# b1xian/arm-neon-opencv

Hardware: AMD Instinct MI355X
Metric: Mpixels/sec per op (resize/warp/normalize) at 1080p; achieved HBM GB/s vs peak (higher is better)
Workload: dtype u8; 1 GPU; resize_normalize INTER_LINEAR 1920x1080x3 u8 NHWC -> 640x360x3 fp32 (reference arithmetic) + per-channel normalize; global_batch=256, batch_per_gpu=256, parallelism=dp1, frame=1920x1080x3, output=640x360x3 fp32, graph=False

## Files before the change

### arm-neon-opencv_amd/csrc/vacv_abi.cpp

```cpp
#pragma clang fp contract(off)

#include <hip/hip_runtime.h>

#include <algorithm>
#include <cfloat>
#include <cmath>
#include <cstdint>
#include <cstdlib>
#include <cstring>
#include <map>
#include <set>
#include <mutex>
#include <tuple>
#include <utility>

#include "vacv_internal.hpp"
#include "vacv_semantics.hpp"

namespace vacv {
namespace {

int esize_of(int dtype) {
    switch (dtype) {
        case VACV_FP32: return 4;
        case VACV_FP16: return 2;
        case VACV_INT8: return 1;
        case VACV_FP64: return 8;
        default: return 0;
    }
}

struct Img {
    unsigned char* data;
    int n, w, h, c, dtype, layout, es;
    int64_t row, plane, batch;
};

int load(const vacv_image* d, Img& m) {
    if (!d || !d->data) return VACV_ERR_INVALID_ARG;
    if (d->n < 1 || d->w < 1 || d->h < 1 || d->c < 1) return VACV_ERR_INVALID_ARG;
    m.es = esize_of(d->dtype);
    if (!m.es) return VACV_ERR_UNSUPPORTED;
    if (d->layout != VACV_NHWC && d->layout != VACV_NCHW) return VACV_ERR_UNSUPPORTED;
    m.data = static_cast<unsigned char*>(d->data);
    m.n = d->n; m.w = d->w; m.h = d->h; m.c = d->c;
    m.dtype = d->dtype; m.layout = d->layout;
    const int64_t min_row = (int64_t)m.w * (m.layout == VACV_NHWC ? m.c : 1) * m.es;
    m.row = d->row_pitch ? d->row_pitch : min_row;
    if (m.row < min_row) return VACV_ERR_INVALID_ARG;
    if (m.layout == VACV_NCHW) {
        const int64_t min_plane = m.row * (m.h - 1) + min_row;
        m.plane = d->plane_pitch ? d->plane_pitch : m.row * m.h;
        if (m.plane < min_plane) return VACV_ERR_INVALID_ARG;
        const int64_t min_batch = m.plane * (m.c - 1) + min_plane;
        m.batch = d->batch_pitch ? d->batch_pitch : m.plane * m.c;
        if (m.n > 1 && m.batch < min_batch) return VACV_ERR_INVALID_ARG;
    } else {
        m.plane = 0;
        const int64_t min_batch = m.row * (m.h - 1) + min_row;
        m.batch = d->batch_pitch ? d->batch_pitch : m.row * m.h;
        if (m.n > 1 && m.batch < min_batch) return VACV_ERR_INVALID_ARG;
    }
    return VACV_OK;
}

int load2(const vacv_image* src_d, const vacv_image* dst_d, Img& src, Img& dst) {
    const int st = load(src_d, src);
    return st ? st : load(dst_d, dst);
}

bool dense(const Img& m) {
    const int64_t row = (int64_t)m.w * (m.layout == VACV_NHWC ? m.c : 1) * m.es;
    if (m.row != row) return false;
    if (m.layout == VACV_NCHW && m.plane != row * m.h) return false;
    const int64_t img = row * m.h * (m.layout == VACV_NCHW ? m.c : 1);
    return m.n == 1 || m.batch == img;
}

PlaneGeom geom(const Img& m) {
    PlaneGeom g;
    g.base = m.data;
    g.img_pitch = m.batch;
    g.row_pitch = m.row;
    g.w = m.w;
    g.h = m.h;
    g.esize = m.es;
    if (m.layout == VACV_NHWC) {
        g.planes = 1;
        g.cc = m.c;
        g.plane_pitch = 0;
    } else {
        g.planes = m.c;
        g.cc = 1;
        g.plane_pitch = m.plane;
    }
    g.plane_bytes = m.row * (m.h - 1) + (int64_t)m.w * g.cc * m.es;
    return g;
}

int hip_status(hipError_t e) { return e == hipSuccess ? VACV_OK : VACV_ERR_HIP; }

bool same_shape(const Img& a, const Img& b) {
    return a.n == b.n && a.w == b.w && a.h == b.h && a.c == b.c && a.layout == b.layout;
}

struct Workspace {
    void* buf = nullptr;
    size_t cap = 0;
};
std::mutex g_ws_mu;
std::map<std::tuple<int, void*, int>, Workspace> g_ws;

int workspace(hipStream_t s, size_t bytes, void** out, int slot = 0, bool zero_new = false) {
    int dev = 0;
    if (hipGetDevice(&dev) != hipSuccess) return VACV_ERR_HIP;
    std::lock_guard<std::mutex> lk(g_ws_mu);
    Workspace& w = g_ws[std::make_tuple(dev, (void*)s, slot)];
    if (w.cap < bytes) {
        if (w.buf) {
            if (hipStreamSynchronize(s) != hipSuccess) return VACV_ERR_HIP;
            (void)hipFree(w.buf);
            w.buf = nullptr;
            w.cap = 0;
        }
        size_t cap = std::max<size_t>(bytes, 1 << 20);
        if (hipMalloc(&w.buf, cap) != hipSuccess) return VACV_ERR_NO_MEMORY;
        w.cap = cap;
        if (zero_new && hipMemsetAsync(w.buf, 0, cap, s) != hipSuccess) return VACV_ERR_HIP;
    }
    *out = w.buf;
    return VACV_OK;
}

size_t align_up(size_t v, size_t a) { return (v + a - 1) / a * a; }

int channel_sums_into(const Img& m, double* sums, int per_image, double* partials, int blocks, hipStream_t s) {
    SumsLaunch L{};
    L.src = geom(m);
    L.n = m.n;
    L.c = m.c;
    L.src_u8 = m.dtype == VACV_INT8;
    L.blocks_per_image = blocks;
    L.partials = partials;
    L.sums = sums;
    L.per_image = per_image;
    L.scalar_only = 0;
    for (int i = 0; i < m.n && !L.scalar_only; ++i)
        for (int p = 0; p < L.src.planes; ++p) {
            uintptr_t a = reinterpret_cast<uintptr_t>(m.data + (int64_t)i * m.batch + (int64_t)p * L.src.plane_pitch);
            if (a & 15) { L.scalar_only = 1; break; }
        }
    return hip_status(launch_channel_sums(L, s));
}

int sums_blocks(const Img& m) {
    const int64_t elems = (int64_t)m.w * m.h * (m.layout == VACV_NHWC ? m.c : 1);
    const int64_t planes = (int64_t)m.n * (m.layout == VACV_NHWC ? 1 : m.c);
    int64_t b = std::max<int64_t>(1, 2048 / std::max<int64_t>(planes, 1));
    b = std::min<int64_t>(b, std::max<int64_t>(1, elems / 4096));
    return (int)std::min<int64_t>(b, 1024);
}

int per_image_stats(const Img& m, hipStream_t s, float** mean, float** stdv) {
    if (m.layout == VACV_NHWC && m.c > 4) return VACV_ERR_UNSUPPORTED;
    if (!dense(m)) return VACV_ERR_UNSUPPORTED;
    const int blocks = sums_blocks(m);
    const int planes = m.layout == VACV_NHWC ? 1 : m.c;
    const int cc = m.layout == VACV_NHWC ? m.c : 1;
    const size_t part_b = align_up((size_t)m.n * planes * blocks * 2 * cc * sizeof(double), 256);
    const size_t sums_b = align_up((size_t)m.n * m.c * 2 * sizeof(double), 256);
    const size_t stat_b = align_up((size_t)m.n * m.c * sizeof(float), 256);
    void* ws = nullptr;
    int st = workspace(s, part_b + sums_b + 2 * stat_b, &ws);
    if (st) return st;
    char* p = static_cast<char*>(ws);
    double* partials = reinterpret_cast<double*>(p);
    double* sums = reinterpret_cast<double*>(p + part_b);
    *mean = reinterpret_cast<float*>(p + part_b + sums_b);
    *stdv = reinterpret_cast<float*>(p + part_b + sums_b + stat_b);
    st = channel_sums_into(m, sums, 1, partials, blocks, s);
    if (st) return st;
    return hip_status(launch_stats(sums, m.n, m.c, (double)m.w * m.h, *mean, *stdv, s));
}

int norm_spec(const Img& shape, const float* mean, const float* stdv, NormSpec& ns) {
    std::memset(&ns, 0, sizeof(ns));
    ns.c_total = shape.c;
    if (!mean && !stdv) return VACV_OK;
    if (!mean || !stdv) return VACV_ERR_INVALID_ARG;
    if (shape.c > kMaxC) return VACV_ERR_UNSUPPORTED;
    ns.mode = 1;
    ns.mul_ok = 0;
    ns.f32_ok = 0;
    for (int k = 0; k < shape.c; ++k) {
        ns.mean[k] = mean[k];
        ns.stdv[k] = stdv[k];
        ns.inv[k] = 1.0 / ((double)stdv[k] + 1e-6);
        ns.inv_hi[k] = (float)ns.inv[k];
        ns.inv_lo[k] = (float)(ns.inv[k] - (double)ns.inv_hi[k]);
        bool ok = true, ok32 = true;
        for (int v = 0; v < 256; ++v) {
            const float d = (float)v - mean[k];
            const float want = normalize_value((float)v, mean[k], stdv[k]);
            ok = ok && (float)((double)d * ns.inv[k]) == want;
            const float lo = d * ns.inv_lo[k];
            const float got = std::fma(d, ns.inv_hi[k], lo);
            ok32 = ok32 && std::memcmp(&got, &want, sizeof(float)) == 0;
        }
        if (ok) ns.mul_ok |= 1u << k;
        if (ok32) ns.f32_ok |= 1u << k;
    }
    return VACV_OK;
}

int normalize_with(const Img& src, const Img& dst, const NormSpec& ns, hipStream_t s) {
    NormLaunch L{};
    L.src = geom(src);
    L.dst = geom(dst);
    L.n = src.n;
    L.src_u8 = src.dtype == VACV_INT8;
    L.norm = ns;
    return hip_status(launch_normalize(L, s));
}

struct FusedSums {
    double* partials;
    double* sums;
    int per_image;
    float* mean;
    float* stddev;
    int groups;
    bool used;
    int64_t* acc;
};

int resolve_out(const Img& src, const Img& dst, int out_kind, int& out) {
    out = (src.dtype == VACV_FP32 && out_kind == kOutF32) ? kOutSame : out_kind;
    const int want = out == kOutSame ? src.dtype : VACV_FP32;
    return dst.dtype == want ? VACV_OK : VACV_ERR_INVALID_ARG;
}

int resize_impl(const vacv_image* src_d, const vacv_image* dst_d, int interpolation, int mode, int out_kind,
                const NormSpec* ns, hipStream_t s, double fx = 0.0, double fy = 0.0, FusedSums* fs = nullptr) {
    Img src, dst;
    int st = load2(src_d, dst_d, src, dst);
    if (st) return st;
    if (src.n != dst.n || src.c != dst.c || src.layout != dst.layout) return VACV_ERR_INVALID_ARG;
    if (src.layout == VACV_NHWC && src.c > 4) return VACV_ERR_UNSUPPORTED;
    if (mode < VACV_LINEAR_REFERENCE || mode > VACV_LINEAR_OPENCV) return VACV_ERR_INVALID_ARG;

    ResizeLaunch L{};
    L.src = geom(src);
    L.dst = geom(dst);
    if (L.src.plane_bytes > kMaxPlaneBytes || L.dst.plane_bytes > kMaxPlaneBytes) return VACV_ERR_UNSUPPORTED;
    L.n = src.n;
    L.mode = mode;
    L.out = out_kind;
    if (ns) L.norm = *ns;
    if (interpolation == VACV_INTER_LINEAR) {
        if (src.w < 2 || src.h < 2) return VACV_ERR_INVALID_ARG;
        if (src.dtype == VACV_INT8) {
            L.kind = kLinearFixed;
            const int want = out_kind == kOutSame ? VACV_INT8 : VACV_FP32;
            if (dst.dtype != want) return VACV_ERR_INVALID_ARG;
        } else if (src.dtype == VACV_FP32) {
            L.kind = kLinearFloat;
            if (dst.dtype != VACV_FP32) return VACV_ERR_INVALID_ARG;
            if (out_kind == kOutF32) L.out = kOutSame;
        } else {
            return VACV_ERR_UNSUPPORTED;
        }
    } else if (interpolation == VACV_INTER_CUBIC) {
        if (src.w < 4 || src.h < 4) return VACV_ERR_INVALID_ARG;
        if (src.dtype != VACV_INT8 && src.dtype != VACV_FP32) return VACV_ERR_UNSUPPORTED;
        if (dst.dtype != VACV_FP32) return VACV_ERR_UNSUPPORTED;
        L.kind = kCubic;
        if (L.out == kOutSame && src.dtype == VACV_INT8) L.out = kOutF32;
        if (L.out == kOutF32 && src.dtype == VACV_FP32) L.out = kOutSame;
    } else if (interpolation == VACV_INTER_NEAREST) {
        if (src.dtype != VACV_INT8 && src.dtype != VACV_FP32) return VACV_ERR_UNSUPPORTED;
        if ((st = resolve_out(src, dst, out_kind, L.out))) return st;
        L.scale_xd = 1. / (fx > 0 ? fx : (double)dst.w / src.w);
        L.scale_yd = 1. / (fy > 0 ? fy : (double)dst.h / src.h);
        return hip_status(launch_resize_nearest(L, s));
    } else if (interpolation == VACV_INTER_AREA) {
        if (src.dtype != VACV_INT8 && src.dtype != VACV_FP32) return VACV_ERR_UNSUPPORTED;
        if ((st = resolve_out(src, dst, out_kind, L.out))) return st;
        const double ifx = fx > 0 ? fx : (double)dst.w / src.w, ify = fy > 0 ? fy : (double)dst.h / src.h;
        const double sx = 1. / ifx, sy = 1. / ify;
        const double ix = std::nearbyint(sx), iy = std::nearbyint(sy);
        if (sx >= 1 && sy >= 1 && std::fabs(sx - ix) < DBL_EPSILON && std::fabs(sy - iy) < DBL_EPSILON) {
            L.area_x = (int)ix;
            L.area_y = (int)iy;
            if ((int64_t)dst.w * L.area_x != src.w || (int64_t)dst.h * L.area_y != src.h) return VACV_ERR_UNSUPPORTED;
            L.area_scale = 1.f / (float)(L.area_x * L.area_y);
            L.area_half_up = src.dtype == VACV_INT8 && L.area_x == 2 && L.area_y == 2 &&
                             (L.src.cc == 1 || L.src.cc == 3 || L.src.cc == 4);
            return hip_status(launch_resize_area(L, s));
        }
        return launch_resize_area_general(L, ifx, ify, s);
    } else if (interpolation == VACV_INTER_LANCZOS4) {
        if (src.dtype != VACV_INT8 && src.dtype != VACV_FP32) return VACV_ERR_UNSUPPORTED;
        if ((st = resolve_out(src, dst, out_kind, L.out))) return st;
        const double ifx = fx > 0 ? fx : (double)dst.w / src.w, ify = fy > 0 ? fy : (double)dst.h / src.h;
        return launch_resize_lanczos(L, ifx, ify, s);
    } else {
        return VACV_ERR_UNSUPPORTED;
    }
    L.scale_xf = (float)src.w / (float)dst.w;
    L.scale_yf = (float)src.h / (float)dst.h;
    L.scale_xd = (double)src.w / (double)dst.w;
    L.scale_yd = (double)src.h / (double)dst.h;
    const int direct = tune_or(VACV_TUNE_RESIZE_DIRECT, 1);
    if (L.kind == kLinearFixed && L.src.cc <= 4 && dst.w < (1 << 23) && dst.h < (1 << 23) &&
        (direct == 2 || ((direct == 1 || direct == 3) && resize_one_tap_rows(L))))
        return hip_status(launch_resize_direct(L, s));
    if (L.kind == kLinearFixed && tune_or(VACV_TUNE_RESIZE_STRIP, 1) >= 1 && resize_strip_applies(L))
        return hip_status(launch_resize_strip(L, s));
    if (cubic_direct_applies(L)) {
        if (fs && L.out == kOutF32 && fs->partials && L.src.planes == 1) {
            L.sum_partials = fs->partials;
            L.sum_out = fs->sums;
            L.sum_per_image = fs->per_image;
            L.sum_mean = fs->mean;
            L.sum_std = fs->stddev;
            L.sum_acc = fs->acc;
            fs->groups = cubic_direct_groups(L);
            fs->used = true;
        }
        return hip_status(launch_cubic_direct(L, s));
    }
    L.interleave = tune(VACV_TUNE_RESIZE_INTERLEAVE) != 0;
    if ((st = plan_resize(L, s))) return st;
    return hip_status(launch_resize(L, s));
}

int copy_rows(const Img& src, const Img& dst, int64_t src_off, int rows_h, int64_t row_bytes, hipStream_t s) {
    CopyLaunch L{};
    L.src = geom(src);
    L.dst = geom(dst);
    L.src.base += src_off;
    L.src.h = rows_h;
    L.n = src.n;
    L.row_bytes = row_bytes;
    return hip_status(launch_row_copy(L, s));
}

int clone_rows(const Img& src, const Img& dst, hipStream_t s) {
    const int cc = src.layout == VACV_NHWC ? src.c : 1;
    return copy_rows(src, dst, 0, src.h, (int64_t)src.w * cc * src.es, s);
}

int dtype_convert(const Img& src, const Img& dst, hipStream_t s) {
    if (!dense(src) || !dense(dst)) return VACV_ERR_UNSUPPORTED;
    DtypeLaunch L{};
    L.src = src.data;
    L.dst = dst.data;
    L.count = (int64_t)src.n * src.w * src.h * src.c;
    L.to_f32 = src.dtype == VACV_INT8;
    return hip_status(launch_dtype(L, s));
}

int border_values(const Img& src, const double* bv, float out[4]) {
    for (int k = 0; k < 4; ++k) {
        const double v = bv ? bv[k] : 0.0;
        if (src.dtype == VACV_INT8) {
            double r = std::nearbyint(v);
            out[k] = (float)std::min(255.0, std::max(0.0, r));
        } else {
            out[k] = (float)v;
        }
    }
    return VACV_OK;
}

int warp_impl(const vacv_image* src_d, const vacv_image* dst_d, const float m[6], int flags, int border_mode,
              const double bv[4], int out_kind, const NormSpec* ns, hipStream_t s) {
    Img src, dst;
    int st = load2(src_d, dst_d, src, dst);
    if (st) return st;
    if (!m) return VACV_ERR_INVALID_ARG;
    if (src.n != dst.n || src.c != dst.c || src.layout != dst.layout) return VACV_ERR_INVALID_ARG;
    if (src.dtype != VACV_INT8 && src.dtype != VACV_FP32) return VACV_ERR_UNSUPPORTED;
    const int interp = flags & 7;
    const bool inverse_map = (flags & VACV_WARP_INVERSE_MAP) != 0;
    if (flags & ~(7 | VACV_WARP_INVERSE_MAP)) return VACV_ERR_UNSUPPORTED;
    if (interp != VACV_INTER_LINEAR && interp != VACV_INTER_NEAREST) return VACV_ERR_UNSUPPORTED;
    if (border_mode < VACV_BORDER_CONSTANT || border_mode > VACV_BORDER_TRANSPARENT) return VACV_ERR_UNSUPPORTED;
    if (src.layout == VACV_NHWC && src.c > 4) return VACV_ERR_UNSUPPORTED;
    if (interp == VACV_INTER_LINEAR && (src.w < 2 || src.h < 2)) return VACV_ERR_INVALID_ARG;
    WarpLaunch L{};
    L.src = geom(src);
    L.dst = geom(dst);
    L.n = src.n;
    if ((st = resolve_out(src, dst, out_kind, L.out))) return st;
    if (inverse_map) std::memcpy(L.inv, m, sizeof(L.inv));
    else vacv_invert_affine(m, L.inv);
    border_values(src, bv, L.border);
    L.border_mode = border_mode;
    if (border_mode == VACV_BORDER_TRANSPARENT && dst.data == src.data) return VACV_ERR_INVALID_ARG;
    if (ns) L.norm = *ns;
    if (interp == VACV_INTER_NEAREST) {
        double* M = L.invd;
        for (int i = 0; i < 6; ++i) M[i] = (double)m[i];
        if (!inverse_map) {
            double D = M[0] * M[4] - M[1] * M[3];
            D = D != 0 ? 1. / D : 0;
            const double A11 = M[4] * D, A22 = M[0] * D;
            M[0] = A11;
            M[1] *= -D;
            M[3] *= -D;
            M[4] = A22;
            const double b1 = -M[0] * M[2] - M[1] * M[5];
            const double b2 = -M[3] * M[2] - M[4] * M[5];
            M[2] = b1;
            M[5] = b2;
        }
        return hip_status(launch_warp_nearest(L, s));
    }
    return hip_status(launch_warp(L, s));
}

int warp_rois_impl(const vacv_image* src_d, const vacv_image* dst_d, const float* m, const int32_t* src_index,
                   int flags, int border_mode, const double bv[4], const NormSpec* ns, hipStream_t s) {
    Img src, dst;
    int st = load2(src_d, dst_d, src, dst);
    if (st) return st;
    if (!m) return VACV_ERR_INVALID_ARG;
    if (src.c != dst.c) return VACV_ERR_INVALID_ARG;
    if (!src_index && src.n != 1 && src.n != dst.n) return VACV_ERR_INVALID_ARG;
    if (src.dtype != VACV_INT8 && src.dtype != VACV_FP32) return VACV_ERR_UNSUPPORTED;
    if (src.layout != VACV_NHWC) return VACV_ERR_UNSUPPORTED;
    if (flags & ~(7 | VACV_WARP_INVERSE_MAP)) return VACV_ERR_UNSUPPORTED;
    if ((flags & 7) != VACV_INTER_LINEAR) return VACV_ERR_UNSUPPORTED;
    if (border_mode < VACV_BORDER_CONSTANT || border_mode >= VACV_BORDER_TRANSPARENT) return VACV_ERR_UNSUPPORTED;
    if (src.c > 4) return VACV_ERR_UNSUPPORTED;
    if (src.w < 2 || src.h < 2) return VACV_ERR_INVALID_ARG;
    if (dst.dtype != (ns ? VACV_FP32 : src.dtype)) return VACV_ERR_INVALID_ARG;
    if (!ns && dst.layout != VACV_NHWC) return VACV_ERR_INVALID_ARG;
    const bool planar = dst.layout == VACV_NCHW && dst.c > 1;
    if (planar && dst.c != 3) return VACV_ERR_UNSUPPORTED;
    WarpRoisLaunch L{};
    L.src = geom(src);
    if (L.src.plane_bytes > kMaxPlaneBytes) return VACV_ERR_UNSUPPORTED;
    L.dst = geom(dst);
    L.n_src = src.n;
    L.n_roi = dst.n;
    L.m = m;
    L.src_index = src_index;
    L.inverse_map = (flags & VACV_WARP_INVERSE_MAP) != 0;
    border_values(src, bv, L.border);
    L.border_mode = border_mode;
    L.out = ns ? kOutNorm : kOutSame;
    L.planar = planar;
    if (ns) L.norm = *ns;
    return hip_status(launch_warp_rois(L, s));
}

int color_code(int code, int& v_first, int& rgb) {
    switch (code) {
        case VACV_COLOR_YUV2BGR_NV21: v_first = 1; rgb = 0; return VACV_OK;
        case VACV_COLOR_YUV2RGB_NV21: v_first = 1; rgb = 1; return VACV_OK;
        case VACV_COLOR_YUV2BGR_NV12: v_first = 0; rgb = 0; return VACV_OK;
        case VACV_COLOR_YUV2RGB_NV12: v_first = 0; rgb = 1; return VACV_OK;
        default: return VACV_ERR_UNSUPPORTED;
    }
}

int color_impl(const vacv_image* src_d, const vacv_image* dst_d, int code, int out_kind, const NormSpec* ns,
               hipStream_t s) {
    Img src, dst;
    int st = load2(src_d, dst_d, src, dst);
    if (st) return st;
    int v_first, rgb;
    if ((st = color_code(code, v_first, rgb))) return st;
    if (src.dtype != VACV_INT8 || src.c != 1) return VACV_ERR_INVALID_ARG;
    const int h = src.h / 3 * 2;
    if (src.w % 2 || h % 2 || h < 2 || src.h != h / 2 * 3) return VACV_ERR_INVALID_ARG;
    if (dst.w != src.w || dst.h != h || dst.c != 3 || dst.layout != VACV_NHWC || dst.n != src.n)
        return VACV_ERR_INVALID_ARG;
    const int want = out_kind == kOutSame ? VACV_INT8 : VACV_FP32;
    if (dst.dtype != want) return VACV_ERR_INVALID_ARG;
    ColorLaunch L{};
    L.src = src.data;
    L.src_img = src.batch;
    L.src_row = src.row;
    L.dst = dst.data;
    L.dst_img = dst.batch;
    L.dst_row = dst.row;
    L.n = src.n;
    L.w = src.w;
    L.h = h;
    L.v_first = v_first;
    L.rgb = rgb;
    L.out = out_kind;
    if (ns) L.norm = *ns;
    return hip_status(launch_color(L, s));
}

int color_cv_impl(const vacv_image* src_d, const vacv_image* dst_d, int code, hipStream_t s) {
    Img src, dst;
    int st = load2(src_d, dst_d, src, dst);
    if (st) return st;
    if (src.layout != VACV_NHWC || dst.layout != VACV_NHWC || src.c != 1 || dst.n != src.n) return VACV_ERR_INVALID_ARG;
    CvColorLaunch L{};
    L.src = src.data;
    L.src_img = src.batch;
    L.src_row = src.row;
    L.dst = dst.data;
    L.dst_img = dst.batch;
    L.dst_row = dst.row;
    L.n = src.n;
    L.w = src.w;
    if (code == VACV_COLOR_GRAY2BGR) {
        if (src.dtype != VACV_INT8 && src.dtype != VACV_FP32) return VACV_ERR_UNSUPPORTED;
        if (dst.dtype != src.dtype || dst.w != src.w || dst.h != src.h || dst.c != 3) return VACV_ERR_INVALID_ARG;
        if (src.es == 4 && ((src.row | dst.row | src.batch | dst.batch) % 4 ||
                            reinterpret_cast<uintptr_t>(src.data) % 4 || reinterpret_cast<uintptr_t>(dst.data) % 4))
            return VACV_ERR_INVALID_ARG;
        L.gray = 1;
        L.h = src.h;
        L.dcn = 3;
        L.esize = src.es;
        return hip_status(launch_color_cv(L, s));
    }
    if (src.dtype != VACV_INT8 || dst.dtype != VACV_INT8) return VACV_ERR_INVALID_ARG;
    const int h = src.h / 3 * 2;
    if (src.w % 2 || h % 2 || h < 2 || src.h != h / 2 * 3) return VACV_ERR_INVALID_ARG;
    L.h = h;
    switch (code) {
        case VACV_COLOR_YUV2RGBA_NV12: L.layout = 0; L.dcn = 4; L.bidx = 2; break;
        case VACV_COLOR_YUV2BGRA_NV12: L.layout = 0; L.dcn = 4; L.bidx = 0; break;
        case VACV_COLOR_YUV2RGBA_NV21: L.layout = 1; L.dcn = 4; L.bidx = 2; break;
        case VACV_COLOR_YUV2BGRA_NV21: L.layout = 1; L.dcn = 4; L.bidx = 0; break;
        default: L.layout = 2; L.dcn = 3; L.bidx = 0; break;
    }
    if (L.layout == 2 && src.row != src.w) return VACV_ERR_INVALID_ARG;
    if (dst.w != src.w || dst.h != h || dst.c != L.dcn) return VACV_ERR_INVALID_ARG;
    const int al = L.dcn == 4 ? 8 : 2;
    L.aligned = !((dst.row | dst.batch) % al) && !(reinterpret_cast<uintptr_t>(dst.data) % al);
    return hip_status(launch_color_cv(L, s));
}

int yuv_resize_impl(const vacv_image* src_d, const vacv_image* dst_d, int code, int interpolation, int mode,
                    int out_kind, const NormSpec* ns, hipStream_t s) {
    Img src, dst;
    int st = load2(src_d, dst_d, src, dst);
    if (st) return st;
    int v_first, rgb;
    if ((st = color_code(code, v_first, rgb))) return st;
    if (interpolation != VACV_INTER_LINEAR) return VACV_ERR_UNSUPPORTED;
    if (mode < VACV_LINEAR_REFERENCE || mode > VACV_LINEAR_OPENCV) return VACV_ERR_INVALID_ARG;
    if (src.dtype != VACV_INT8 || src.c != 1 || src.layout != VACV_NHWC) return VACV_ERR_INVALID_ARG;
    const int h = src.h / 3 * 2;
    if (src.w % 2 || h % 2 || h < 2 || src.w < 4 || src.h != h / 2 * 3) return VACV_ERR_INVALID_ARG;
    if (dst.c != 3 || dst.n != src.n) return VACV_ERR_INVALID_ARG;
    const int want = out_kind == kOutSame ? VACV_INT8 : VACV_FP32;
    if (dst.dtype != want) return VACV_ERR_INVALID_ARG;
    const int64_t src_bytes = src.row * (src.h - 1) + src.w;
    const int64_t P = (int64_t)dst.w * dst.h;
    if (src_bytes > kMaxPlaneBytes || P > 0x7FFFFFFFLL - 1024 || src.n > 65535) return VACV_ERR_UNSUPPORTED;
    YuvResizeLaunch L{};
    L.src = src.data;
    L.src_img = src.batch;
    L.src_row = src.row;
    L.src_bytes = src_bytes;
    L.dst = dst.data;
    L.dst_img = dst.batch;
    L.dst_row = dst.row;
    L.dst_plane = dst.plane;
    L.n = src.n;
    L.w = src.w;
    L.h = h;
    L.wo = dst.w;
    L.ho = dst.h;
    L.v_first = v_first;
    L.rgb = rgb;
    L.chw = dst.layout == VACV_NCHW;
    L.mode = mode;
    L.out = out_kind;
    L.scale_xf = (float)L.w / (float)L.wo;
    L.scale_yf = (float)L.h / (float)L.ho;
    L.scale_xd = (double)L.w / (double)L.wo;
    L.scale_yd = (double)L.h / (double)L.ho;
    if (ns) L.norm = *ns;
    return hip_status(launch_yuv_resize(L, s));
}

int fused_normalize(const vacv_image* dst_d, const float* mean, const float* stddev, hipStream_t s,
                    int (*pass)(const void*, int, const NormSpec*, hipStream_t), const void* ctx) {
    Img dst;
    int st = load(dst_d, dst);
    if (st) return st;
    if (dst.dtype != VACV_FP32) return VACV_ERR_INVALID_ARG;
    NormSpec ns;
    if ((st = norm_spec(dst, mean, stddev, ns))) return st;
    if (ns.mode == 1) return pass(ctx, kOutNorm, &ns, s);
    if ((st = pass(ctx, kOutF32, nullptr, s))) return st;
    float *dm = nullptr, *ds = nullptr;
    if ((st = per_image_stats(dst, s, &dm, &ds))) return st;
    ns.mode = 2;
    ns.dev_mean = dm;
    ns.dev_std = ds;
    return normalize_with(dst, dst, ns, s);
}

struct ResizeCtx {
    const vacv_image* src;
    const vacv_image* dst;
    int interpolation, mode;
};
int resize_pass(const void* c, int out, const NormSpec* ns, hipStream_t s) {
    const ResizeCtx* r = static_cast<const ResizeCtx*>(c);
    return resize_impl(r->src, r->dst, r->interpolation, r->mode, out, ns, s);
}

struct WarpCtx {
    const vacv_image* src;
    const vacv_image* dst;
// ... 447 lines not shown
```

### arm-neon-opencv_amd/csrc/vacv_internal.hpp

```cpp
#pragma once

#include <hip/hip_runtime.h>
#include <cstdint>
#include <set>

#include "../../include/vacv_hip.h"

namespace vacv {

constexpr int kBlock = 256;
constexpr int kMaxC = VACV_MAX_CHANNELS;
constexpr int kResizeMaxChunksPerLane = 1;
constexpr int64_t kMaxPlaneBytes = 0x7FFFFFF0LL;

int tune(int key);
inline int tune_or(int key, int def) {
    const int v = tune(key);
    return v < 0 ? def : v;
}

struct PlaneGeom {
    const unsigned char* base;
    int64_t img_pitch;
    int64_t plane_pitch;
    int64_t row_pitch;
    int planes;
    int w, h;
    int cc;
    int esize;
    int64_t plane_bytes;
};

struct NormSpec {
    int mode;
    int c_total;
    const float* dev_mean;
    const float* dev_std;
    float mean[kMaxC];
    float stdv[kMaxC];
    double inv[kMaxC];
    uint32_t mul_ok;
    float inv_hi[kMaxC];
    float inv_lo[kMaxC];
    uint32_t f32_ok;
};

enum SampleKind : int {
    kLinearFixed = 0,
    kLinearFloat = 1,
    kCubic = 2,
};

enum OutKind : int {
    kOutSame = 0,
    kOutF32 = 1,
    kOutNorm = 2,
};

struct ResizePlanDev {
    const int* xoff;
    const void* xw;
    const int* col_first;
    const int* cpr;
    const int* yrow;
    const void* yw;
    const int* task_nslots;
    const int* task_rows;
    const int* task_cand;
    const int* task_flags;
    const float* lut;
};

struct ResizeLaunch {
    PlaneGeom src;
    PlaneGeom dst;
    int n;
    int kind;
    int mode;
    int out;
    float scale_xf, scale_yf;
    double scale_xd, scale_yd;
    int tile_w, tile_h, tiles_x, tiles_y;
    int sparse;
    int max_slots;
    int slot_stride;
    int lds_bytes;
    int strips;
    int tasks_per_strip;
    int interleave;
    int area_x, area_y;
    float area_scale;
    int area_half_up;
    ResizePlanDev plan;
    NormSpec norm;
    double* sum_partials;
    double* sum_out;
    int sum_per_image;
    float* sum_mean;
    float* sum_std;
    int64_t* sum_acc;
    int sum_q1, sum_q2;
};

int plan_resize(ResizeLaunch& L, hipStream_t s);
void set_strips(ResizeLaunch& L, int64_t resident_workgroups);
int release_plans();

template <class Map, class FreeFn>
int evict_device_cache(Map& m, FreeFn free_entry) {
    int cur = 0, st = VACV_OK;
    if (hipGetDevice(&cur) != hipSuccess) st = VACV_ERR_HIP;
    std::set<int> owners;
    for (auto& kv : m) owners.insert(kv.second.device);
    for (int d : owners)
        if (hipSetDevice(d) != hipSuccess || hipDeviceSynchronize() != hipSuccess) st = VACV_ERR_HIP;
    for (auto& kv : m)
        if (hipSetDevice(kv.second.device) != hipSuccess || !free_entry(kv.second)) st = VACV_ERR_HIP;
    if (!m.empty() && hipSetDevice(cur) != hipSuccess) st = VACV_ERR_HIP;
    m.clear();
    return st;
}

hipError_t launch_resize(const ResizeLaunch& L, hipStream_t s);
hipError_t launch_resize_direct(const ResizeLaunch& L, hipStream_t s);
bool resize_one_tap_rows(const ResizeLaunch& L);
bool resize_strip_applies(const ResizeLaunch& L);
hipError_t launch_resize_strip(const ResizeLaunch& L, hipStream_t s);
hipError_t launch_resize_nearest(const ResizeLaunch& L, hipStream_t s);
hipError_t launch_resize_area(const ResizeLaunch& L, hipStream_t s);
int launch_resize_area_general(const ResizeLaunch& L, double inv_x, double inv_y, hipStream_t s);
int release_area_tables();
int launch_resize_lanczos(const ResizeLaunch& L, double inv_x, double inv_y, hipStream_t s);
int release_lanczos_tables();
bool cubic_direct_applies(const ResizeLaunch& L);
hipError_t launch_cubic_direct(const ResizeLaunch& L, hipStream_t s);
int cubic_direct_groups(const ResizeLaunch& L);
int64_t cubic_sums_groups_bound(int w, int h);

struct WarpLaunch {
    PlaneGeom src;
    PlaneGeom dst;
    int n;
    float inv[6];
    double invd[6];
    float border[4];
    int border_mode;
    int out;
    NormSpec norm;
};
hipError_t launch_warp(const WarpLaunch& L, hipStream_t s);
hipError_t launch_warp_nearest(const WarpLaunch& L, hipStream_t s);
struct WarpRoisLaunch {
    PlaneGeom src;
    PlaneGeom dst;
    int n_src, n_roi;
    const float* m;
    const int32_t* src_index;
    int inverse_map;
    float border[4];
    int border_mode;
    int out;
    int planar;
    NormSpec norm;
};
hipError_t launch_warp_rois(const WarpRoisLaunch& L, hipStream_t s);
hipError_t launch_invert_affine(const float* m, float* inv, int n, hipStream_t s);
struct WarpFramesPlan {
    int th;
    int S;
    int rows_max;
    int ns;
    int slot;
    int lds;
    int kf;
    int dst_al;
    int se;
    int raw_bytes;
    int exp_units;
    int tw;
};
bool warp_frames_plan(const WarpLaunch& L, WarpFramesPlan& P);
hipError_t launch_warp_frames(const WarpLaunch& L, const WarpFramesPlan& P, hipStream_t s);
bool warp_exp_nn_plan(const WarpLaunch& L, WarpFramesPlan& P);
hipError_t launch_warp_exp_nn(const WarpLaunch& L, const WarpFramesPlan& P, hipStream_t s);

struct CopyLaunch {
    PlaneGeom src;
    PlaneGeom dst;
    int n;
    int64_t row_bytes;
};
hipError_t launch_row_copy(const CopyLaunch& L, hipStream_t s);

struct LayoutLaunch {
    const unsigned char* src;
    unsigned char* dst;
    int n, w, h, c, esize;
    int to_chw;
    int64_t src_img, dst_img;
};
hipError_t launch_layout(const LayoutLaunch& L, hipStream_t s);

struct DtypeLaunch {
    const unsigned char* src;
    unsigned char* dst;
    int64_t count;
    int to_f32;
};
hipError_t launch_dtype(const DtypeLaunch& L, hipStream_t s);
hipError_t launch_u8_to_f32_rows(const CopyLaunch& L, hipStream_t s);

struct ColorLaunch {
    const unsigned char* src;
    int64_t src_img, src_row;
    unsigned char* dst;
    int64_t dst_img, dst_row;
    int n, w, h;
    int v_first;
    int rgb;
    int out;
    NormSpec norm;
};
hipError_t launch_color(const ColorLaunch& L, hipStream_t s);

struct CvColorLaunch {
    const unsigned char* src;
    int64_t src_img, src_row;
    unsigned char* dst;
    int64_t dst_img, dst_row;
    int n, w, h;
    int gray;
    int layout;
    int dcn;
    int bidx;
    int esize;
    int aligned;
};
hipError_t launch_color_cv(const CvColorLaunch& L, hipStream_t s);

struct YuvResizeLaunch {
    const unsigned char* src;
    int64_t src_img, src_row;
    int64_t src_bytes;
    unsigned char* dst;
    int64_t dst_img, dst_row, dst_plane;
    int n, w, h;
    int wo, ho;
    int v_first;
    int rgb;
    int chw;
    int mode;
    int out;
    float scale_xf, scale_yf;
    double scale_xd, scale_yd;
    NormSpec norm;
};
hipError_t launch_yuv_resize(const YuvResizeLaunch& L, hipStream_t s);

struct NormLaunch {
    PlaneGeom src;
    PlaneGeom dst;
    int n;
    int src_u8;
    NormSpec norm;
};
hipError_t launch_normalize(const NormLaunch& L, hipStream_t s);

struct SumsLaunch {
    PlaneGeom src;
    int n;
    int c;
    int src_u8;
    int blocks_per_image;
    double* partials;
    double* sums;
    int per_image;
    int scalar_only;
};
hipError_t launch_channel_sums(const SumsLaunch& L, hipStream_t s);
hipError_t launch_stats(const double* sums, int groups, int c, double count,
                        float* mean, float* stddev, hipStream_t s);

struct MatchLaunch {
    const unsigned char* img;
    int64_t img_pitch, img_row;
    int iw, ih, cn, esize, n;
    const unsigned char* tpl;
    int64_t tpl_row;
    int tw, th;
    unsigned char* res;
    int64_t res_pitch, res_row;
    int rw, rh;
    int method;
    double inv_area;
    double* box;
    double* tstats;
    void* bfrag;
};
size_t match_lds_bytes(int tw, int th, int cn, int esize);
bool match_mfma_plan(int tw, int th, int cn, int& KB, int& stride);
size_t match_bfrag_bytes(int tw, int th, int cn);
hipError_t launch_match_template(const MatchLaunch& M, hipStream_t s);

struct MinMaxLaunch {
    const unsigned char* src;
    int64_t row;
    int w, h, esize;
    const unsigned char* mask;
    int64_t mask_row;
    double* out_val;
    int* out_idx;
};
size_t min_max_workspace_bytes();
hipError_t launch_min_max(const MinMaxLaunch& L, void* ws, hipStream_t s);

}
```

Measured before the change: 2.586 million Mpixels/s.

## Add rational-ratio block resize kernel with register taps and LDS-staged stores

Adds a resize path for integer-ratio downscales (3:2, 2:1). Each wave loads a block of source rows into registers with one buffer load per lane and row, builds the bilinear taps with byte-permute, and stages the output through per-wave LDS so it can be written as coalesced 128-bit stores. It is selected by default for fixed-point linear resizes whose output is not u8, taking precedence over the strip kernel. This trades more template instantiations and register/LDS pressure for fewer redundant gathers and better-coalesced stores.

```diff
diff --git a/arm-neon-opencv_amd/csrc/k_resize_block.hip b/arm-neon-opencv_amd/csrc/k_resize_block.hip
--- /dev/null
+++ b/arm-neon-opencv_amd/csrc/k_resize_block.hip
@@ -0,0 +1,346 @@
+#pragma clang fp contract(off)
+
+#include "vacv_device.hpp"
+
+namespace vacv {
+namespace {
+
+#ifndef VACV_BLOCK_ROWS
+#define VACV_BLOCK_ROWS 2
+#endif
+#ifndef VACV_BLOCK_LAUX
+#define VACV_BLOCK_LAUX 2
+#endif
+#ifndef VACV_BLOCK_ROUND
+#define VACV_BLOCK_ROUND 6144
+#endif
+constexpr int kBlockRows = VACV_BLOCK_ROWS;
+
+constexpr int block_tap(int p, int q, int r) { return ((2 * r + 1) * p - q) / (2 * q); }
+
+constexpr bool block_lines(int cc, int p) { return p * cc == 9; }
+
+constexpr int block_round_rows(int rows, int row_bytes) {
+    int g = rows;
+    while (g > 1 && g * row_bytes > VACV_BLOCK_ROUND) g /= 2;
+    return g;
+}
+
+template <int B0, int B1>
+__device__ __forceinline__ uint32_t byte_pair(const uint32_t (&d)[3]) {
+    constexpr int w0 = B0 / 4, w1 = B1 / 4;
+    static_assert(w1 < 3 && (w1 == w0 || w1 > w0), "taps inside the lane's load");
+    constexpr uint32_t sel = (uint32_t)(B0 % 4) | (0x0Cu << 8) | ((uint32_t)((w1 == w0 ? 0 : 4) + B1 % 4) << 16) |
+                             (0x0Cu << 24);
+    return __builtin_amdgcn_perm(d[w1], d[w0], sel);
+}
+
+template <class F, int... Is>
+__device__ __forceinline__ void static_for_seq(F&& f, std::integer_sequence<int, Is...>) {
+    (f(std::integral_constant<int, Is>()), ...);
+}
+template <int N, class F>
+__device__ __forceinline__ void static_for(F&& f) {
+    static_for_seq(f, std::make_integer_sequence<int, N>());
+}
+
+[[maybe_unused]] constexpr int block_waves(int out, int cw, int lds_bytes) {
+    const int by_lds = 160 * 1024 / lds_bytes;
+    const int by_regs = out != kOutNorm ? 8 : cw == 2 ? 5 : 6;
+    return by_lds < by_regs ? by_lds : by_regs;
+}
+template <int CC, int OUT, int Q, int CW>
+constexpr int block_lds_bytes() {
+    constexpr int row = 64 * CW * Q * CC * (OUT == kOutSame ? 1 : 4);
+    return 4 * block_round_rows(Q * kBlockRows, row) * row;
+}
+
+template <int CC, int OUT, int MODE, int P, int Q, int CW>
+__global__ void __launch_bounds__(kBlock)
+__attribute__((amdgpu_waves_per_eu(block_waves(OUT, CW, block_lds_bytes<CC, OUT, Q, CW>()))))
+resize_block_kernel(ResizeLaunch L, int col_blocks, int row_groups, int tasks, int dst16) {
+    constexpr int R = kBlockRows;
+    using TOut = typename std::conditional<(OUT == kOutSame), uint8_t, float>::type;
+    constexpr int kOutPx = CC * (int)sizeof(TOut);
+    constexpr int kSrcB = P * CC;
+    constexpr int ND = (kSrcB + 3) / 4;
+    static_assert(ND <= 3, "one load per lane and row");
+    constexpr bool kLines = CW == 2;
+    static_assert(!kLines || block_lines(CC, P), "CW = 2 is the line-exact path");
+    constexpr int kLoadAux = kLines ? VACV_BLOCK_LAUX : 0;
+    constexpr int kStoreAux = VACV_STORE_AUX;
+    constexpr uint32_t kShift = kLines ? (uint32_t)(4 * ND - kSrcB) : 0u;
+    constexpr int kCols = 64 * CW * Q;
+    constexpr int kRowB = kCols * kOutPx;
+    constexpr int G = block_round_rows(Q * R, kRowB);
+    __shared__ __attribute__((aligned(16))) unsigned char xch[4][G * kRowB];
+    const int lane = (int)threadIdx.x & 63;
+    const int wave = __builtin_amdgcn_readfirstlane((int)threadIdx.x >> 6);
+    const int task = (int)blockIdx.x * 4 + wave;
+    if (task >= tasks) return;
+    const int per_plane = col_blocks * row_groups;
+    const int pidx = task / per_plane;
+    const int rem = task - pidx * per_plane;
+    const int rg = rem / col_blocks, cb = rem - rg * col_blocks;
+    const int img = pidx / L.src.planes, plane = pidx - img * L.src.planes;
+    const int W = L.dst.w, H = L.dst.h;
+    const int nbx = W / Q;
+    const int kb0 = cb * 64 * CW;
+    const int x0 = kb0 * Q, y0 = rg * R * Q;
+    const int ncol = min(kCols, W - x0);
+    const int nrow = min(R * Q, H - y0);
+    const int sy0 = rg * R * P;
+    const int nsrc = min(R * P, L.src.h - sy0);
+
+    const unsigned char* sp = L.src.base + (int64_t)img * L.src.img_pitch + (int64_t)plane * L.src.plane_pitch;
+    const Rsrc srs = make_rsrc(sp, L.src.plane_bytes);
+    const uint32_t slimit = (uint32_t)L.src.plane_bytes + srs.delta;
+    const uint32_t rp = (uint32_t)L.src.row_pitch;
+
+    us2 wx[CW][Q];
+    uint32_t xoff[CW];
+    const uint32_t tsh = kLines && lane == 63 ? kShift : 0u;
+#pragma unroll
+    for (int c = 0; c < CW; ++c) {
+        const int kb = min(kb0 + 64 * c + lane, nbx - 1);
+#pragma unroll
+        for (int j = 0; j < Q; ++j) {
+            const FixedTap tx = tap_of<MODE>(kb * Q + j, L.src.w, W, L.scale_xf, L.scale_xd);
+            wx[c][j] = __builtin_bit_cast(us2, (uint32_t)tx.w0 | ((uint32_t)tx.w1 << 16));
+            if (j == 0) xoff[c] = (uint32_t)((tx.i - block_tap(P, Q, 0)) * CC) + srs.delta - (c == CW - 1 ? tsh : 0u);
+        }
+    }
+    uint32_t my_w = 0;
+    if (lane < Q * R) {
+        const FixedTap ty = tap_of<MODE>(min(y0 + lane, H - 1), L.src.h, H, L.scale_yf, L.scale_yd);
+        my_w = (uint32_t)ty.w0 | ((uint32_t)ty.w1 << 16);
+    }
+
+    uint32_t d[R * P][CW][3];
+    const uint32_t last_ro = (uint32_t)(sy0 + nsrc - 1) * rp;
+    const bool safe = __builtin_amdgcn_ballot_w64(last_ro + xoff[CW - 1] + 4u * ND > slimit ||
+                                                  last_ro + xoff[0] + 4u * ND > slimit) == 0;
+    auto gather = [&](auto safe_c) {
+        constexpr bool SAFE = decltype(safe_c)::value;
+#pragma unroll
+        for (int i = 0; i < R * P; ++i) {
+            const uint32_t ro = (uint32_t)(sy0 + i) * rp;
+#pragma unroll
+            for (int c = 0; c < CW; ++c) {
+                d[i][c][0] = d[i][c][1] = d[i][c][2] = 0u;
+                if (i >= nsrc) continue;
+                const uint32_t o = ro + xoff[c];
+                if (SAFE || o + 4u * ND <= slimit) {
+                    if constexpr (ND == 1) {
+                        d[i][c][0] = (uint32_t)__builtin_amdgcn_raw_buffer_load_b32(srs.r, (int)o, 0, kLoadAux);
+                    } else if constexpr (ND == 2) {
+                        const auto v = __builtin_amdgcn_raw_buffer_load_b64(srs.r, (int)o, 0, kLoadAux);
+                        d[i][c][0] = v[0];
+                        d[i][c][1] = v[1];
+                    } else {
+                        const auto v = __builtin_amdgcn_raw_buffer_load_b96(srs.r, (int)o, 0, kLoadAux);
+                        d[i][c][0] = v[0];
+                        d[i][c][1] = v[1];
+                        d[i][c][2] = v[2];
+                    }
+                } else {
+                    const uint32_t sh = c == CW - 1 ? tsh : 0u;
+                    const unsigned char* b = sp + (int64_t)(o - srs.delta);
+#pragma unroll
+                    for (int e = 0; e < 4 * ND; ++e)
+                        if (e >= (int)sh && e < (int)sh + kSrcB) d[i][c][e >> 2] |= (uint32_t)b[e] << (8 * (e & 3));
+                }
+            }
+        }
+    };
+    if (safe) gather(std::true_type());
+    else gather(std::false_type());
+
+    ChanNorm cn[CC] = {};
+    if (OUT == kOutNorm) {
+#pragma unroll
+        for (int k = 0; k < CC; ++k) cn[k] = chan_norm(L.norm, img, CC == 1 ? plane % L.norm.c_total : k);
+    }
+    unsigned char* dp = const_cast<unsigned char*>(L.dst.base) + (int64_t)img * L.dst.img_pitch +
+                        (int64_t)plane * L.dst.plane_pitch;
+    const Rsrc rd = make_rsrc(dp, L.dst.plane_bytes);
+    const bool full = ncol == kCols && dst16;
+    TOut* xo = reinterpret_cast<TOut*>(xch[wave]);
+    const unsigned char* xs = xch[wave];
+    const uint32_t drp = (uint32_t)L.dst.row_pitch;
+
+    bool norm32 = OUT == kOutNorm;
+#pragma unroll
+    for (int k = 0; k < CC; ++k) norm32 = norm32 && cn[k].f32;
+    auto rounds = [&](auto n32) {
+    constexpr bool N32 = decltype(n32)::value;
+    static_for<Q * R / G>([&](auto gc) {
+        constexpr int g = decltype(gc)::value;
+        const int rows = min(G, nrow - g * G);
+        if (rows <= 0) return;
+        static_for<G>([&](auto tc) {
+            constexpr int t = decltype(tc)::value;
+            constexpr int oy = g * G + t;
+            constexpr int ia = (oy / Q) * P + block_tap(P, Q, oy % Q);
+            if constexpr (kLines) {
+                constexpr int seen = oy == 0 ? 0 : ((oy - 1) / Q) * P + block_tap(P, Q, (oy - 1) % Q) + 2;
+                static_for<ia + 2 - seen>([&](auto ic) {
+                    uint32_t(&v)[3] = d[seen + decltype(ic)::value][CW - 1];
+                    v[0] = __builtin_amdgcn_alignbyte(v[1], v[0], tsh);
+                    v[1] = __builtin_amdgcn_alignbyte(v[2], v[1], tsh);
+                    v[2] = __builtin_amdgcn_alignbyte(0u, v[2], tsh);
+                });
+            }
+            const uint32_t wr = (uint32_t)__builtin_amdgcn_readlane((int)my_w, oy);
+            const uint32_t wA = wr & 0xFFFFu, wB = wr >> 16;
+            static_for<CW>([&](auto cc_) {
+                constexpr int c = decltype(cc_)::value;
+                TOut vals[Q * CC];
+                static_for<Q>([&](auto jc) {
+                    constexpr int j = decltype(jc)::value;
+                    constexpr int lx = block_tap(P, Q, j);
+                    static_for<CC>([&](auto kc) {
+                        constexpr int k = decltype(kc)::value;
+                        const uint32_t top = byte_pair<lx * CC + k, (lx + 1) * CC + k>(d[ia][c]);
+                        const uint32_t bot = byte_pair<lx * CC + k, (lx + 1) * CC + k>(d[ia + 1][c]);
+                        const int v = blend_fixed<MODE>(top, bot, wx[c][j], wA, wB);
+                        if constexpr (N32) {
+                            const float df = (float)v - cn[k].mean;
+                            vals[j * CC + k] = (TOut)__builtin_fmaf(df, cn[k].hi, df * cn[k].lo);
+                        } else {
+                            vals[j * CC + k] = emit_u8<OUT, TOut>(cn[k], v);
+                        }
+                    });
+                });
+                TOut* o = xo + (t * 64 * CW + 64 * c + lane) * Q * CC;
+#pragma unroll
+                for (int e = 0; e < Q * CC; ++e) o[e] = vals[e];
+            });
+        });
+        wave_lds_sync();
+        const uint32_t base = (uint32_t)(y0 + g * G) * drp + (uint32_t)(x0 * kOutPx) + rd.delta;
+        if (full) {
+            constexpr int kCpr = kRowB / 16;
+            for (int ch = lane; ch < rows * kCpr; ch += 64) {
+                const int rr = ch / kCpr, cc = ch - rr * kCpr;
+                __builtin_amdgcn_raw_buffer_store_b128(*reinterpret_cast<const u32x4*>(xs + 16 * ch), rd.r,
+                                                       (int)(base + (uint32_t)rr * drp + 16u * cc), 0, kStoreAux);
+            }
+        } else {
+            const int rb = ncol * kOutPx;
+            for (int e = lane; e < rows * rb; e += 64) {
+                const int rr = e / rb, cc = e - rr * rb;
+                __builtin_amdgcn_raw_buffer_store_b8(xs[rr * kRowB + cc], rd.r, (int)(base + (uint32_t)rr * drp + cc), 0,
+                                                     kStoreAux);
+            }
+        }
+        wave_lds_sync();
+    });
+    };
+    if (OUT == kOutNorm && norm32) rounds(std::true_type());
+    else rounds(std::false_type());
+}
+
+constexpr int kRatios[][2] = {{3, 2}, {2, 1}};
+
+bool block_taps(int n_in, int n_out, float sf, double sd, int mode, int p, int q) {
+    for (int dd = 0; dd < n_out; ++dd) {
+        const int k = dd / q, r = dd - k * q;
+        if (fixed_tap(dd, n_in, n_out, sf, sd, mode).i != p * k + block_tap(p, q, r)) return false;
+    }
+    return true;
+}
+
+bool block_ratio(const ResizeLaunch& L, int& p, int& q) {
+    for (const auto& pq : kRatios) {
+        p = pq[0];
+        q = pq[1];
+        if ((int64_t)L.src.w * q == (int64_t)L.dst.w * p && (int64_t)L.src.h * q == (int64_t)L.dst.h * p) return true;
+    }
+    return false;
+}
+
+int block_cw(const ResizeLaunch& L, int p, int q) {
+    if (!block_lines(L.src.cc, p) || (L.dst.w / q) % 128) return 1;
+    const bool lines = L.src.row_pitch % 128 == 0 && (reinterpret_cast<uintptr_t>(L.src.base) & 127) == 0 &&
+                       L.src.img_pitch % 128 == 0 && L.src.plane_pitch % 128 == 0;
+    return lines ? 2 : 1;
+}
+
+int64_t block_tasks(const ResizeLaunch& L, int p, int q, int cw, int& col_blocks, int& row_groups) {
+    col_blocks = (L.dst.w / q + 64 * cw - 1) / (64 * cw);
+    row_groups = (L.dst.h / q + kBlockRows - 1) / kBlockRows;
+    return (int64_t)col_blocks * row_groups * L.n * L.src.planes;
+}
+
+template <int CC, int OUT, int MODE, int P, int Q>
+hipError_t launch_one(const ResizeLaunch& L, hipStream_t s) {
+    const int cw = block_cw(L, P, Q);
+    int col_blocks = 0, row_groups = 0;
+    const int64_t tasks = block_tasks(L, P, Q, cw, col_blocks, row_groups);
+    const uintptr_t dbits = reinterpret_cast<uintptr_t>(L.dst.base) | (uintptr_t)L.dst.row_pitch |
+                            (uintptr_t)L.dst.img_pitch | (uintptr_t)L.dst.plane_pitch;
+    const int dst16 = (dbits & 15) == 0;
+    const unsigned grid = (unsigned)((tasks + 3) / 4);
+    if constexpr (block_lines(CC, P)) {
+        if (cw == 2) {
+            hipLaunchKernelGGL((resize_block_kernel<CC, OUT, MODE, P, Q, 2>), dim3(grid), dim3(kBlock), 0, s, L,
+                               col_blocks, row_groups, (int)tasks, dst16);
+            return hipGetLastError();
+        }
+    }
+    hipLaunchKernelGGL((resize_block_kernel<CC, OUT, MODE, P, Q, 1>), dim3(grid), dim3(kBlock), 0, s, L, col_blocks,
+                       row_groups, (int)tasks, dst16);
+    return hipGetLastError();
+}
+
+template <int CC, int OUT, int MODE>
+hipError_t launch_ratio(const ResizeLaunch& L, int p, hipStream_t s) {
+    return p == 3 ? launch_one<CC, OUT, MODE, 3, 2>(L, s) : launch_one<CC, OUT, MODE, 2, 1>(L, s);
+}
+
+template <int OUT, int MODE>
+hipError_t launch_cc(const ResizeLaunch& L, int p, hipStream_t s) {
+    switch (L.src.cc) {
+        case 1: return launch_ratio<1, OUT, MODE>(L, p, s);
+        case 2: return launch_ratio<2, OUT, MODE>(L, p, s);
+        case 3: return launch_ratio<3, OUT, MODE>(L, p, s);
+        case 4: return launch_ratio<4, OUT, MODE>(L, p, s);
+        default: return hipErrorInvalidValue;
+    }
+}
+
+template <int OUT>
+hipError_t launch_mode(const ResizeLaunch& L, int p, hipStream_t s) {
+    switch (L.mode) {
+        case VACV_LINEAR_REFERENCE: return launch_cc<OUT, VACV_LINEAR_REFERENCE>(L, p, s);
+        case VACV_LINEAR_NEON: return launch_cc<OUT, VACV_LINEAR_NEON>(L, p, s);
+        case VACV_LINEAR_OPENCV: return launch_cc<OUT, VACV_LINEAR_OPENCV>(L, p, s);
+        default: return hipErrorInvalidValue;
+    }
+}
+
+}
+
+bool resize_block_applies(const ResizeLaunch& L) {
+    if (L.kind != kLinearFixed || L.src.esize != 1 || L.src.cc < 1 || L.src.cc > 4) return false;
+    if (L.mode != VACV_LINEAR_REFERENCE && L.mode != VACV_LINEAR_NEON && L.mode != VACV_LINEAR_OPENCV) return false;
+    if (L.dst.w >= (1 << 23) || L.dst.h >= (1 << 23)) return false;
+    if (L.src.plane_bytes > kMaxPlaneBytes || L.dst.plane_bytes > kMaxPlaneBytes) return false;
+    int p, q;
+    if (!block_ratio(L, p, q)) return false;
+    int col_blocks, row_groups;
+    if (block_tasks(L, p, q, 1, col_blocks, row_groups) >= 0x7FFFFFF0LL) return false;
+    return block_taps(L.src.w, L.dst.w, L.scale_xf, L.scale_xd, L.mode, p, q) &&
+           block_taps(L.src.h, L.dst.h, L.scale_yf, L.scale_yd, L.mode, p, q);
+}
+
+hipError_t launch_resize_block(const ResizeLaunch& L, hipStream_t s) {
+    int p, q;
+    if (!resize_block_applies(L) || !block_ratio(L, p, q)) return hipErrorInvalidValue;
+    if (L.out == kOutSame) return launch_mode<kOutSame>(L, p, s);
+    if (L.out == kOutF32) return launch_mode<kOutF32>(L, p, s);
+    return launch_mode<kOutNorm>(L, p, s);
+}
+
+}
diff --git a/arm-neon-opencv_amd/csrc/vacv_abi.cpp b/arm-neon-opencv_amd/csrc/vacv_abi.cpp
--- a/arm-neon-opencv_amd/csrc/vacv_abi.cpp
+++ b/arm-neon-opencv_amd/csrc/vacv_abi.cpp
@@ -315,6 +315,11 @@
     if (L.kind == kLinearFixed && L.src.cc <= 4 && dst.w < (1 << 23) && dst.h < (1 << 23) &&
         (direct == 2 || ((direct == 1 || direct == 3) && resize_one_tap_rows(L))))
         return hip_status(launch_resize_direct(L, s));
+    const int strip = tune(VACV_TUNE_RESIZE_STRIP);
+    if (L.kind == kLinearFixed && (strip == 3 || (strip < 0 && L.out != kOutSame))) {
+        if (resize_block_applies(L)) return hip_status(launch_resize_block(L, s));
+        if (strip == 3) return VACV_ERR_INVALID_ARG;
+    }
     if (L.kind == kLinearFixed && tune_or(VACV_TUNE_RESIZE_STRIP, 1) >= 1 && resize_strip_applies(L))
         return hip_status(launch_resize_strip(L, s));
     if (cubic_direct_applies(L)) {
diff --git a/arm-neon-opencv_amd/csrc/vacv_internal.hpp b/arm-neon-opencv_amd/csrc/vacv_internal.hpp
--- a/arm-neon-opencv_amd/csrc/vacv_internal.hpp
+++ b/arm-neon-opencv_amd/csrc/vacv_internal.hpp
@@ -126,6 +126,8 @@
 bool resize_one_tap_rows(const ResizeLaunch& L);
 bool resize_strip_applies(const ResizeLaunch& L);
 hipError_t launch_resize_strip(const ResizeLaunch& L, hipStream_t s);
+bool resize_block_applies(const ResizeLaunch& L);
+hipError_t launch_resize_block(const ResizeLaunch& L, hipStream_t s);
 hipError_t launch_resize_nearest(const ResizeLaunch& L, hipStream_t s);
 hipError_t launch_resize_area(const ResizeLaunch& L, hipStream_t s);
 int launch_resize_area_general(const ResizeLaunch& L, double inv_x, double inv_y, hipStream_t s);
```

Measured after the change: 2.586 million Mpixels/s, median of 3. About the same (+0.0%).
